# TinyMPC/TinyMPC

Hardware: AMD Instinct MI355X
Metric: QP solves/sec (+ ADMM iters/sec), 64k-batch quadrotor hover (higher is better)
Workload: dtype f64; 1 GPU; quadrotor_hovering (nx=12, nu=4, N=10), 65536 identical instances per GPU, closed-loop MPC steps from a cold start (BASELINE configs[1]); batch_per_gpu=65536, total_batch=65536, parallelism=batch-sharded x1, mpc_steps_per_launch=8, stats_exchange=none (one rank), launcher=plain process

## Files before the change

### tinympc_amd/csrc/admm_kernel.hip.h

```cpp
#pragma once
#include <hip/hip_runtime.h>
#include <stdint.h>

namespace tinympc_amd {

enum : int {
    TAB_MB = 0,
    TAB_MF1 = 256,
    TAB_MF2 = 512,
    TAB_PT = 768,
    TAB_VEC = 1024,
    TAB_BOUNDS = 1024 + 16 * 16,
};
enum : int {
    VEC_CB = 0,
    VEC_CF = 1,
    VEC_QR = 2,
    VEC_SMASK = 3,
    VEC_NIM = 4,
    VEC_SOCFLAG = 5,
    VEC_CONE_BASE = 6,
    VEC_CONE_MU = 7,
    VEC_LINFLAG = 9,
    VEC_TLINFLAG = 10,
// ... 385 lines not shown
#define HAH7 HAH6 "v_fmac_f64_dpp %[acc], %[sa], %[a6] row_newbcast:8+6 row_mask:0xf bank_mask:0xc\n\t"
#define HAH8 HAH7 "v_fmac_f64_dpp %[acc], %[sa], %[a7] row_newbcast:8+7 row_mask:0xf bank_mask:0xc\n\t"
#define HBL1 "v_fmac_f64_dpp %[acc], %[sb], %[b0] row_newbcast:%[c0]+0 row_mask:0xf bank_mask:0x3\n\t"
#define HBL2 HBL1 "v_fmac_f64_dpp %[acc], %[sb], %[b1] row_newbcast:%[c0]+1 row_mask:0xf bank_mask:0x3\n\t"
#define HBL3 HBL2 "v_fmac_f64_dpp %[acc], %[sb], %[b2] row_newbcast:%[c0]+2 row_mask:0xf bank_mask:0x3\n\t"
#define HBL4 HBL3 "v_fmac_f64_dpp %[acc], %[sb], %[b3] row_newbcast:%[c0]+3 row_mask:0xf bank_mask:0x3\n\t"
#define HBL5 HBL4 "v_fmac_f64_dpp %[acc], %[sb], %[b4] row_newbcast:%[c0]+4 row_mask:0xf bank_mask:0x3\n\t"
#define HBL6 HBL5 "v_fmac_f64_dpp %[acc], %[sb], %[b5] row_newbcast:%[c0]+5 row_mask:0xf bank_mask:0x3\n\t"
#define HBL7 HBL6 "v_fmac_f64_dpp %[acc], %[sb], %[b6] row_newbcast:%[c0]+6 row_mask:0xf bank_mask:0x3\n\t"
#define HBL8 HBL7 "v_fmac_f64_dpp %[acc], %[sb], %[b7] row_newbcast:%[c0]+7 row_mask:0xf bank_mask:0x3\n\t"
#define HBH1 "v_fmac_f64_dpp %[acc], %[sb], %[b0] row_newbcast:8+%[c0]+0 row_mask:0xf bank_mask:0xc\n\t"
#define HBH2 HBH1 "v_fmac_f64_dpp %[acc], %[sb], %[b1] row_newbcast:8+%[c0]+1 row_mask:0xf bank_mask:0xc\n\t"
#define HBH3 HBH2 "v_fmac_f64_dpp %[acc], %[sb], %[b2] row_newbcast:8+%[c0]+2 row_mask:0xf bank_mask:0xc\n\t"
#define HBH4 HBH3 "v_fmac_f64_dpp %[acc], %[sb], %[b3] row_newbcast:8+%[c0]+3 row_mask:0xf bank_mask:0xc\n\t"
#define HBH5 HBH4 "v_fmac_f64_dpp %[acc], %[sb], %[b4] row_newbcast:8+%[c0]+4 row_mask:0xf bank_mask:0xc\n\t"
#define HBH6 HBH5 "v_fmac_f64_dpp %[acc], %[sb], %[b5] row_newbcast:8+%[c0]+5 row_mask:0xf bank_mask:0xc\n\t"
#define HBH7 HBH6 "v_fmac_f64_dpp %[acc], %[sb], %[b6] row_newbcast:8+%[c0]+6 row_mask:0xf bank_mask:0xc\n\t"
#define HBH8 HBH7 "v_fmac_f64_dpp %[acc], %[sb], %[b7] row_newbcast:8+%[c0]+7 row_mask:0xf bank_mask:0xc\n\t"
#define HFAL1 "v_fmac_f64_dpp %[t], %[xi], %[a0] row_newbcast:0 row_mask:0xf bank_mask:0x3\n\t"
#define HFAL2 HFAL1 "v_fmac_f64_dpp %[t], %[xi], %[a1] row_newbcast:1 row_mask:0xf bank_mask:0x3\n\t"
#define HFAL3 HFAL2 "v_fmac_f64_dpp %[t], %[xi], %[a2] row_newbcast:2 row_mask:0xf bank_mask:0x3\n\t"
#define HFAL4 HFAL3 "v_fmac_f64_dpp %[t], %[xi], %[a3] row_newbcast:3 row_mask:0xf bank_mask:0x3\n\t"
#define HFAL5 HFAL4 "v_fmac_f64_dpp %[t], %[xi], %[a4] row_newbcast:4 row_mask:0xf bank_mask:0x3\n\t"
#define HFAL6 HFAL5 "v_fmac_f64_dpp %[t], %[xi], %[a5] row_newbcast:5 row_mask:0xf bank_mask:0x3\n\t"
#define HFAL7 HFAL6 "v_fmac_f64_dpp %[t], %[xi], %[a6] row_newbcast:6 row_mask:0xf bank_mask:0x3\n\t"
#define HFAL8 HFAL7 "v_fmac_f64_dpp %[t], %[xi], %[a7] row_newbcast:7 row_mask:0xf bank_mask:0x3\n\t"
#define HFAH1 "v_fmac_f64_dpp %[t], %[xi], %[a0] row_newbcast:8+0 row_mask:0xf bank_mask:0xc\n\t"
#define HFAH2 HFAH1 "v_fmac_f64_dpp %[t], %[xi], %[a1] row_newbcast:8+1 row_mask:0xf bank_mask:0xc\n\t"
#define HFAH3 HFAH2 "v_fmac_f64_dpp %[t], %[xi], %[a2] row_newbcast:8+2 row_mask:0xf bank_mask:0xc\n\t"
#define HFAH4 HFAH3 "v_fmac_f64_dpp %[t], %[xi], %[a3] row_newbcast:8+3 row_mask:0xf bank_mask:0xc\n\t"
#define HFAH5 HFAH4 "v_fmac_f64_dpp %[t], %[xi], %[a4] row_newbcast:8+4 row_mask:0xf bank_mask:0xc\n\t"
#define HFAH6 HFAH5 "v_fmac_f64_dpp %[t], %[xi], %[a5] row_newbcast:8+5 row_mask:0xf bank_mask:0xc\n\t"
#define HFAH7 HFAH6 "v_fmac_f64_dpp %[t], %[xi], %[a6] row_newbcast:8+6 row_mask:0xf bank_mask:0xc\n\t"
#define HFAH8 HFAH7 "v_fmac_f64_dpp %[t], %[xi], %[a7] row_newbcast:8+7 row_mask:0xf bank_mask:0xc\n\t"
#define HFBL1 "v_fmac_f64_dpp %[xn], %[t], %[b0] row_newbcast:%[c0]+0 row_mask:0xf bank_mask:0x3\n\t"
#define HFBL2 HFBL1 "v_fmac_f64_dpp %[xn], %[t], %[b1] row_newbcast:%[c0]+1 row_mask:0xf bank_mask:0x3\n\t"
#define HFBL3 HFBL2 "v_fmac_f64_dpp %[xn], %[t], %[b2] row_newbcast:%[c0]+2 row_mask:0xf bank_mask:0x3\n\t"
#define HFBL4 HFBL3 "v_fmac_f64_dpp %[xn], %[t], %[b3] row_newbcast:%[c0]+3 row_mask:0xf bank_mask:0x3\n\t"
#define HFBL5 HFBL4 "v_fmac_f64_dpp %[xn], %[t], %[b4] row_newbcast:%[c0]+4 row_mask:0xf bank_mask:0x3\n\t"
#define HFBL6 HFBL5 "v_fmac_f64_dpp %[xn], %[t], %[b5] row_newbcast:%[c0]+5 row_mask:0xf bank_mask:0x3\n\t"
#define HFBL7 HFBL6 "v_fmac_f64_dpp %[xn], %[t], %[b6] row_newbcast:%[c0]+6 row_mask:0xf bank_mask:0x3\n\t"
#define HFBL8 HFBL7 "v_fmac_f64_dpp %[xn], %[t], %[b7] row_newbcast:%[c0]+7 row_mask:0xf bank_mask:0x3\n\t"
#define HFBH1 "v_fmac_f64_dpp %[xn], %[t], %[b0] row_newbcast:8+%[c0]+0 row_mask:0xf bank_mask:0xc\n\t"
#define HFBH2 HFBH1 "v_fmac_f64_dpp %[xn], %[t], %[b1] row_newbcast:8+%[c0]+1 row_mask:0xf bank_mask:0xc\n\t"
#define HFBH3 HFBH2 "v_fmac_f64_dpp %[xn], %[t], %[b2] row_newbcast:8+%[c0]+2 row_mask:0xf bank_mask:0xc\n\t"
#define HFBH4 HFBH3 "v_fmac_f64_dpp %[xn], %[t], %[b3] row_newbcast:8+%[c0]+3 row_mask:0xf bank_mask:0xc\n\t"
#define HFBH5 HFBH4 "v_fmac_f64_dpp %[xn], %[t], %[b4] row_newbcast:8+%[c0]+4 row_mask:0xf bank_mask:0xc\n\t"
#define HFBH6 HFBH5 "v_fmac_f64_dpp %[xn], %[t], %[b5] row_newbcast:8+%[c0]+5 row_mask:0xf bank_mask:0xc\n\t"
#define HFBH7 HFBH6 "v_fmac_f64_dpp %[xn], %[t], %[b6] row_newbcast:8+%[c0]+6 row_mask:0xf bank_mask:0xc\n\t"
#define HFBH8 HFBH7 "v_fmac_f64_dpp %[xn], %[t], %[b7] row_newbcast:8+%[c0]+7 row_mask:0xf bank_mask:0xc\n\t"
#define FUSED_HBWD_CASE(NA_, NB_) FUSED_HBWD_CASE_(NA_, NB_)
#define FUSED_HBWD_CASE_(NA_, NB_)                                                                                      \
    if constexpr (NA == NA_ && NB == NB_) {                                                                             \
        asm("v_fma_f64 %[qlo], -%[rho], %[tmp], %[qx]\n\t"                                                              \
            "v_fma_f64 %[acc], %[qlo], %[smask], %[cb]\n\t"                                                             \
            "v_fma_f64 %[dnp], %[sa], %[nim], %[cf]\n\t" HAL##NA_ HBL##NB_                                              \
            "v_add_f64 %[tmpn], %[vnn], -%[gn]\n\t" HAH##NA_ HBH##NB_                                                   \
            : [qlo] "=&v"(qlo), [acc] "=&v"(acc), [dnp] "=&v"(dnp), [tmpn] "=&v"(tmpn)                                  \
            : [tmp] "v"(tmp), [vnn] "v"(vnn), [gn] "v"(gn), [qx] "v"(qx), [rho] "v"(rho), [smask] "v"(smask), [cb] "v"(cb), \
              [nim] "v"(nim), [cf] "v"(cf), [sa] "v"(sa), [sb] "v"(sb), [c0] "i"(NA_), FMA##NA_, FMB##NB_);             \
    }
#define FUSED_HFWD_CASE(NA_, NB_) FUSED_HFWD_CASE_(NA_, NB_)
#define FUSED_HFWD_CASE_(NA_, NB_)                                                                                      \
    if constexpr (NA == NA_ && NB == NB_) {                                                                             \
        asm("v_add_f64 %[tt], %[xi], %[g]\n\t"                                                                          \
            "v_max_f64 %[vm], %[lo], %[tt]\n\t" HFAL##NA_                                                               \
            "v_min_f64 %[vn], %[hi], %[vm]\n\t" HFAH##NA_                                                               \
            "v_mov_b64 %[xn], %[t]\n\t"                                                                                 \
            "v_add_f64 %[gnew], %[tt], -%[vn]\n\t" HFBL##NB_                                                            \
            "s_nop 0\n\t" HFBH##NB_                                                                                     \
            : [tt] "=&v"(tt), [vm] "=&v"(vm), [vn] "=&v"(vn), [xn] "=&v"(xn), [t] "+&v"(t), [gnew] "=&v"(gnew)           \
            : [xi] "v"(xi), [g] "v"(g), [lo] "v"(lo), [hi] "v"(hi), [c0] "i"(NA_), FMA##NA_, FMB##NB_);                  \
    }
#if defined(TINYMPC_FUSED_NX) && defined(TINYMPC_FUSED_NU)
#define FUSED_SHAPES(CASE) CASE(TINYMPC_FUSED_NX, TINYMPC_FUSED_NU)
constexpr bool fused_shape(int na, int nb) { return na == TINYMPC_FUSED_NX && nb == TINYMPC_FUSED_NU; }
#if TINYMPC_FUSED_NX + TINYMPC_FUSED_NU <= 8
#define FUSED_HALF_SHAPES(CASE) CASE(TINYMPC_FUSED_NX, TINYMPC_FUSED_NU)
#else
#define FUSED_HALF_SHAPES(CASE)
#endif
#else
#define FUSED_SHAPES(CASE)
#define FUSED_HALF_SHAPES(CASE)
constexpr bool fused_shape(int, int) { return false; }
#endif
template <int NA, int NB>
__device__ __forceinline__ void fused_backward_step(double& qlo, double& acc, double vn, double g, double qx, double rho, double smask, double cb,
                                                    double sa, double sb, const double* ma, const double* mb_) {
    double tmp;
    FUSED_SHAPES(FUSED_BWD_CASE)
    (void)tmp;
}
template <int NA, int NB>
__device__ __forceinline__ void fused_backward_step_soc(double& qlo, double& acc, double vn, double g, double qx, double w, double rho,
                                                        double smask, double cb, double sa, double sb, const double* ma, const double* mb_) {
    double tmp;
    FUSED_SHAPES(FUSED_BWD_SOC_CASE)
    (void)tmp;
}
template <int NA, int NB>
__device__ __forceinline__ void fused_backward_step_half(double& qlo, double& acc, double& dnp, double& tmpn, double tmp, double vnn, double gn, double qx,
                                                         double rho, double smask, double cb, double nim, double cf, double sa, double sb,
                                                         const double* ma, const double* mb_) {
    FUSED_HALF_SHAPES(FUSED_HBWD_CASE)
}
template <int NA, int NB>
__device__ __forceinline__ void fused_forward_step_half(double& tt, double& vn, double& t, double& xn, double& gnew, double xi, double g,
                                                        double lo, double hi, const double* ma, const double* mb_) {
    double vm;
    FUSED_HALF_SHAPES(FUSED_HFWD_CASE)
    (void)vm;
}
template <int NA, int NB, bool INPLACE = false>
__device__ __forceinline__ void fused_forward_step(double& tt, double& vn, double& t, double& xn, double xi, double g, double lo, double hi,
                                                   const double* ma, const double* mb_) {
    double vm;
    FUSED_SHAPES(FUSED_FWD_CASE)
    (void)vm;
}

__device__ __forceinline__ double vmax64(double a, double b) {
    double r;
    asm("v_max_f64 %0, %1, %2" : "=v"(r) : "v"(a), "v"(b));
    return r;
}
__device__ __forceinline__ double vmin64(double a, double b) {
    double r;
    asm("v_min_f64 %0, %1, %2" : "=v"(r) : "v"(a), "v"(b));
    return r;
}
__device__ __forceinline__ double pinned_sub64(double a, double b) {
    double r = a - b;
    asm volatile("" : "+v"(r));
    return r;
}
__device__ __forceinline__ double vclamp64(double lo, double hi, double t) {
    double r;
    asm("v_max_f64 %0, %1, %2\n\tv_min_f64 %0, %3, %0" : "=&v"(r) : "v"(lo), "v"(t), "v"(hi));
    return r;
}

__device__ __forceinline__ double vmax_abs64(double a, double b) {
    double r;
    asm("v_max_f64 %0, %1, |%2|" : "=v"(r) : "v"(a), "v"(b));
    return r;
}
template <bool OPAQUE>
__device__ __forceinline__ double resid_max(double a, double b) {
    if constexpr (OPAQUE) return vmax_abs64(a, b);
    else return fmax(a, fabs(b));
}

#ifndef TINYMPC_PRIM_STORE
#define TINYMPC_PRIM_STORE 1
#endif
#ifndef TINYMPC_REF_LOAD
#define TINYMPC_REF_LOAD 1
#endif
#ifndef TINYMPC_FULL_LINE_STORES
#define TINYMPC_FULL_LINE_STORES 2
#endif
__device__ __forceinline__ double load_ref(const double* p) {
#if TINYMPC_REF_LOAD == 1
    return __builtin_nontemporal_load(p);
#else
    return *p;
#endif
}
__device__ __forceinline__ void store_primal(double* p, double v) {
#if TINYMPC_PRIM_STORE == 1
    __builtin_nontemporal_store(v, p);
#elif TINYMPC_PRIM_STORE == 2
    asm volatile("global_store_dwordx2 %0, %1, off sc1" : : "v"(p), "v"(v) : "memory");
#elif TINYMPC_PRIM_STORE == 3
    asm volatile("global_store_dwordx2 %0, %1, off sc0 sc1" : : "v"(p), "v"(v) : "memory");
#elif TINYMPC_PRIM_STORE == 4
    asm volatile("global_store_dwordx2 %0, %1, off sc0 sc1 nt" : : "v"(p), "v"(v) : "memory");
#else
    *p = v;
#endif
}

__device__ __forceinline__ double grp_max16(double v) {
#pragma unroll
    for (int off = 8; off >= 1; off >>= 1) v = fmax(v, __shfl_xor(v, off, 16));
    return v;
}
template <int W>
__device__ __forceinline__ double grp_maxw(double v) {
#pragma unroll
    for (int off = W / 2; off >= 1; off >>= 1) v = fmax(v, __shfl_xor(v, off, W));
    return v;
}

__device__ __forceinline__ double soc_component(double s0, double s1, double s2, double mine, int c, float mu) {
#pragma clang fp contract(off)
    const double u0 = s2 * (double)mu;
    const double q0 = s0 * s0, q1 = s1 * s1;
    const double q = q0 + q1;
    const bool sure_inside = (u0 > 1e-30) && (q <= (u0 * u0) * (1.0 - 0x1p-20)) && (q < 1e70);
    if (__builtin_amdgcn_ballot_w64(!sure_inside) == 0ull) return mine;
    const float a = (float)sqrt(q);
    const double ad = (double)a;
    const bool below = ad <= -u0, inside = ad <= u0;
    const bool outside = !below && !inside && (ad >= fabs(u0));
    double r = (below || !inside) ? 0.0 : mine;
    if (__builtin_amdgcn_ballot_w64(outside) != 0ull) {
        const double scale = 0.5 * (1.0 + u0 / ad);
        const double last = (double)(a / mu);
        const double o = scale * ((c == 2) ? last : mine);
        r = outside ? o : r;
    }
    return r;
}

__device__ __forceinline__ bool soc_all_inside(double s0, double s1, double s2, float mu) {
#pragma clang fp contract(off)
    const double u0 = s2 * (double)mu;
    const double q0 = s0 * s0, q1 = s1 * s1;
    const double q = q0 + q1;
    const bool sure_inside = (u0 > 1e-30) & (u0 < 1e300) & (q <= (u0 * u0) * (1.0 - 0x1p-20)) & (q < 1e70);
    return __builtin_amdgcn_ballot_w64(!sure_inside) == 0ull;
}
__device__ __forceinline__ void soc_project3(double s0, double s1, double s2, float mu, float rmu, bool rmu_exact, double& r0, double& r1, double& r2) {
#pragma clang fp contract(off)
    const double u0 = s2 * (double)mu;
    const double q0 = s0 * s0, q1 = s1 * s1;
    const double q = q0 + q1;
    const float a = (float)sqrt(q);
    const double ad = (double)a;
    const bool below = ad <= -u0, inside = ad <= u0;
    const bool outside = !below && !inside && (ad >= fabs(u0));
    const bool zero = below || !inside;
    r0 = zero ? 0.0 : s0; r1 = zero ? 0.0 : s1; r2 = zero ? 0.0 : s2;
    if (__builtin_amdgcn_ballot_w64(outside) != 0ull) {
        const double scale = 0.5 * (1.0 + u0 / ad);
        const double last = (double)(rmu_exact ? a * rmu : a / mu);
        r0 = outside ? scale * s0 : r0;
        r1 = outside ? scale * s1 : r1;
        r2 = outside ? scale * last : r2;
    }
}
__device__ __forceinline__ int soc_items_of(unsigned heads, int nx, int n) {
    int c = 0;
    for (unsigned m = heads; m; m &= m - 1) c += (__builtin_ctz(m) < nx) ? n : n - 1;
    return c;
}
constexpr int soc_item_passes(int nx, int nu, int n) { return ((nx / 3) * n + (nu / 3) * (n - 1) + 15) / 16; }

constexpr int ADAPT_LOG = 32;
__device__ __forceinline__ double taylor_step(double a, double d, double b) {
#pragma clang fp contract(off)
    const double t = d * b;
    return a + t;
}

constexpr int solve_kernel_waves_per_simd(int nz, int n, bool soc, bool lin = false, bool adapt = false) {
    if (lin) return 1;
    if (adapt) return n <= 10 ? 2 : 1;
    return (n <= 10 || 2 * ((soc ? 8 : 6) * n + 2 * nz + 8) + 40 <= 256) ? 2 : 1;
}

#ifndef TINYMPC_LIN_WAVES
#define TINYMPC_LIN_WAVES 0
#endif
constexpr long solve_kernel_lin_lds(int nx, int nu, int n, bool soc, int lin, int kmax, bool ub) {
    const int nz = nx + nu, csl = (nz + 1) | 1, cs = (nz + 1) | 1;
    return 8L * (nx * 16 + (ub ? 2 : 2 * n * 16) + ((lin & 1) ? 3 * kmax * 16 + 2 * 4 * n * csl : 0) +
                 ((lin & 2) ? 3 * n * kmax * 16 + 2 * 4 * n * csl : 0) + (soc ? (4 * n + 1) * 3 * cs : 0));
}
constexpr bool solve_kernel_lin_planes(int nx, int nu, int n, bool soc, int lin, int kmax, bool ub) {
    return lin != 0 && solve_kernel_lin_lds(nx, nu, n, soc, lin, kmax, ub) <= 64 * 1024 - 512;
}
constexpr int solve_kernel_lin_waves(int nx, int nu, int n, bool soc, int lin, int kmax, bool ub) {
    if (!solve_kernel_lin_planes(nx, nu, n, soc, lin, kmax, ub)) return 1;
    if (TINYMPC_LIN_WAVES > 0) return TINYMPC_LIN_WAVES;
    return (solve_kernel_waves_per_simd(nx + nu, n, soc) == 2 && 8 * solve_kernel_lin_lds(nx, nu, n, soc, lin, kmax, ub) <= 158 * 1024) ? 2 : 1;
}
template <int NF, int KMAX_, int LW_, int LPI_>
__device__ __forceinline__ void project_halfspace_columns(const int t, const int inst, const int n, const int csl, const int R0, const int S0,
                                                          double* pv, double* pg, const double* tab, const int tab_stride, const int nk) {
#pragma clang fp contract(off)
    for (int c = S0 + t; c < n; c += LPI_) {
        const int at = (inst * n + c) * csl + R0;
        const double* tk = tab + c * tab_stride;
        double z[NF], t0[NF];
#pragma unroll
        for (int r = 0; r < NF; ++r) { z[r] = pv[at + r]; t0[r] = z[r]; }
        for (int k = 0; k < nk; ++k) {
            double cv = 0.0;
#pragma unroll
            for (int r = 0; r < NF; ++r) { const double pr = tk[k * LW_ + R0 + r] * z[r]; cv = cv + pr; }
            const double bk = tk[KMAX_ * LW_ + k * LW_ + R0];
            if (cv > bk) {
                const double dist = (cv - bk) / tk[2 * KMAX_ * LW_ + k * LW_ + R0];
#pragma unroll
                for (int r = 0; r < NF; ++r) { const double pr = dist * tk[k * LW_ + R0 + r]; z[r] = z[r] - pr; }
            }
        }
#pragma unroll
        for (int r = 0; r < NF; ++r) { pv[at + r] = z[r]; pg[at + r] = t0[r] - z[r]; }
    }
}

template <int NX, int NU, int N, bool SOC, bool DBG, int MODE, int LIN = 0, bool HET = false, int KMAX = LIN_KMAX, bool ADAPT = false, bool UB = false, bool HALF = false,
// ... 274 lines not shown
            const int cw = grp * N * SLOT_D + (j < NZ ? j : NZ);
            const double x0v_in = is_state ? (PF ? pf_x0 : P.x0[(size_t)b * NX + j]) : 0.0;
            const int cl = grp * N * CSL + (j < NZ ? j : NZ);
            double VL[LSR ? N : 1], GL[LSR ? N : 1], VT[LTR ? N : 1], GT[LTR ? N : 1];
            double Qd[DBG ? N : 1], Pd[DBG ? N : 1], Dd[DBG ? N : 1];
            double ref_last = 0.0, qx_last_plain = 0.0;
#pragma unroll
            for (int s = 0; s < N; ++s) {
                const bool valid = is_state || (is_input && s >= 1);
                const size_t off = lbase + s * NZ;
                const bool warm = valid && !P.cold;
                if constexpr (PF) {
                    VN[s] = warm ? pfVN[s] : 0.0;
                    G[s] = warm ? pfG[s] : 0.0;
                    VP[s] = warm ? pfVP[s] : 0.0;
                    QX[s] = pfQXs[s];
                    X[s] = 0.0;
                    if (s == N - 1) ref_last = pf_rl;
                    continue;
                }
                const double r = valid ? (P.ref_shared ? P.ref[off - (size_t)b * (N * NZ)] : load_ref(P.ref + off)) : 0.0;
                VN[s] = warm ? P.slack[off] : 0.0;
                G[s] = warm ? P.dual[off] : 0.0;
                VP[s] = warm ? P.slack_prev[off] : 0.0;
                QX[s] = -(r * qr);
                X[s] = 0.0;
                if (s == N - 1) ref_last = r;
                if constexpr (SOC) {
                    double vc0 = (warm && soc_lane) ? (resumed ? P.cslack : P.prim)[off] : 0.0;
                    const double gc0 = (warm && soc_lane) ? P.cdual[off] : 0.0;
                    if (s == 0 && is_state && soc_lane && !resumed) vc0 = x0v_in;
                    sC[cw + s * SLOT_D] = vc0 - gc0;
                    sC[cw + s * SLOT_D + PL_GC] = gc0;
                    sC[cw + s * SLOT_D + PL_VC] = vc0;
                }
                if constexpr (LS) {
                    const double vl0 = (warm && lin_lane) ? (resumed ? P.lslack : P.prim)[off] : 0.0;
                    const double gl0 = (warm && lin_lane) ? P.ldual[off] : 0.0;
                    if constexpr (LSP) { sLV[cl + s * CSL] = vl0; sLG[cl + s * CSL] = gl0; } else { VL[s] = vl0; GL[s] = gl0; }
                }
                if constexpr (LT) {
                    const double vt0 = (warm && tlin_lane) ? (resumed ? P.tlslack : P.prim)[off] : 0.0;
                    const double gt0 = (warm && tlin_lane) ? P.tldual[off] : 0.0;
                    if constexpr (LTP) { sTV[cl + s * CSL] = vt0; sTG[cl + s * CSL] = gt0; } else { VT[s] = vt0; GT[s] = gt0; }
                }
                if constexpr (DBG) { Qd[s] = 0.0; Pd[s] = 0.0; Dd[s] = 0.0; }
            }
            double x0v = x0v_in;
            auto terminal_term = [&]() {
                double pt[NX];
#pragma unroll
                for (int k = 0; k < NX; ++k)
                    pt[k] = ADAPT ? sP[grp * NX * NX + k + NX * (is_state ? j : 0)] : (HET ? het[TAB_PT + k * 16 + j] : sPt[k * 16 + j]);
                double xp = 0.0;
                if constexpr (HALF) ring1_half<0, NX>(xp, ref_last, pt);
                else xp = ring_sum<MODE, 0, NX>(0.0, ref_last, pt);
                qx_last_plain = QX[N - 1];
                QX[N - 1] = is_state ? -xp : QX[N - 1];
            };
            int ndl = 0;
            auto flush_c = [&](int n) {
                __builtin_amdgcn_fence(__ATOMIC_RELEASE, "wavefront");
                __builtin_amdgcn_wave_barrier();
                if (P.aC2 && is_state) {
                    double* c2 = P.aC2 + (size_t)b * (NX * NX) + NX * j;
                    double v[NX], d[NX];
#pragma unroll
                    for (int k = 0; k < NX; ++k) { v[k] = c2[k]; d[k] = P.atab[ATAB_DC2 + k * 16 + j]; }
                    for (int i = 0; i < n; ++i) {
                        const double dl = sDl[grp * ADAPT_LOG + i];
#pragma unroll
                        for (int k = 0; k < NX; ++k) v[k] = taylor_step(v[k], dl, d[k]);
                    }
#pragma unroll
                    for (int k = 0; k < NX; ++k) c2[k] = v[k];
                }
                if (P.aC1 && j < NU) {
                    double* c1 = P.aC1 + (size_t)b * (NU * NU) + NU * j;
                    double v[NU], d[NU];
#pragma unroll
                    for (int k = 0; k < NU; ++k) { v[k] = c1[k]; d[k] = P.atab[ATAB_DC1 + k * 16 + j]; }
                    for (int i = 0; i < n; ++i) {
                        const double dl = sDl[grp * ADAPT_LOG + i];
#pragma unroll
                        for (int k = 0; k < NU; ++k) v[k] = taylor_step(v[k], dl, d[k]);
                    }
#pragma unroll
                    for (int k = 0; k < NU; ++k) c1[k] = v[k];
                }
            };
            if (!has_traj && !(PF && P.ref_shared)) terminal_term();
            const int traj_k0 = has_traj ? (P.traj_step0 + (P.traj_offsets ? P.traj_offsets[b] : 0)) : 0;

            int iter = 0, solved = 0, checked = 0;
            unsigned acc_iter = 0, acc_solved = 0;
            bool vp_touched = false;
            double rp = 0.0, rd = 0.0;
            const int nsteps = PF ? 1 : (P.steps > 1 ? P.steps : 1);
            const int iter_first = resumed ? P.iter_base : 0;
            for (int step = 0; step < nsteps; ++step) {
                X[0] = x0v;
                if (has_traj) {
                    if (is_state) {
#pragma unroll
                        for (int s = 0; s < N; ++s) {
                            int kk = traj_k0 + step + s;
                            kk = kk < P.traj_points ? kk : P.traj_points - 1;
                            const double r = P.traj[(size_t)kk * NX + j];
                            QX[s] = -(r * qr);
                            if (s == N - 1) ref_last = r;
                        }
                    }
                    terminal_term();
                }
                if (P.reset_duals) {
#pragma unroll
                    for (int s = 0; s < N; ++s) G[s] = 0.0;
                }
                if constexpr (SOC) {
                    if (step > 0) {
#pragma unroll
                        for (int s = 0; s < N; ++s) {
                            const double vc0 = soc_lane ? X[s] : 0.0;
                            sC[cw + s * SLOT_D] = vc0 - sC[cw + s * SLOT_D + PL_GC];
                            sC[cw + s * SLOT_D + PL_VC] = vc0;
                        }
                    }
                }
                if constexpr (LS) {
                    if (step > 0) {
#pragma unroll
                        for (int s = 0; s < N; ++s) { if constexpr (LSP) sLV[cl + s * CSL] = lin_lane ? X[s] : 0.0; else VL[s] = lin_lane ? X[s] : 0.0; }
                    } else if (is_state && lin_lane && !resumed) { if constexpr (LSP) sLV[cl] = x0v; else VL[0] = x0v; }
                }
                if constexpr (LT) {
                    if (step > 0) {
#pragma unroll
                        for (int s = 0; s < N; ++s) { if constexpr (LTP) sTV[cl + s * CSL] = tlin_lane ? X[s] : 0.0; else VT[s] = tlin_lane ? X[s] : 0.0; }
                    } else if (is_state && tlin_lane && !resumed) { if constexpr (LTP) sTV[cl] = x0v; else VT[0] = x0v; }
                }
                if constexpr (LPL) __builtin_amdgcn_fence(__ATOMIC_RELEASE, "wavefront");
                const int iter0 = iter_first;
                iter = iter0; solved = 0;
                if (resumed && P.check_termination > 0) checked = 1;
                int countdown = P.check_termination;
                double wr[SOC ? SPR : 1];
                bool gcz[SOC_PASSES];
#pragma unroll
                for (int p = 0; p < SOC_PASSES; ++p) gcz[p] = false;
                if constexpr (SOC) {
#pragma unroll
                    for (int d = 1; d <= SPR && d <= N; ++d) wr[(N - d) % SPR] = sC[cw + (N - d) * SLOT_D];
                }
                for (int it = iter0; it < P.max_iter; ++it) {
                    double lvr[LSP ? SPR : 1], lgr[LSP ? SPR : 1], tvr[LTP ? SPR : 1], tgr[LTP ? SPR : 1];
                    if constexpr (LPL) {
#pragma unroll
                        for (int d = 1; d <= SPR && d <= N; ++d) {
                            if constexpr (LSP) { lvr[(N - d) % SPR] = sLV[cl + (N - d) * CSL]; lgr[(N - d) % SPR] = sLG[cl + (N - d) * CSL]; }
                            if constexpr (LTP) { tvr[(N - d) % SPR] = sTV[cl + (N - d) * CSL]; tgr[(N - d) % SPR] = sTG[cl + (N - d) * CSL]; }
                        }
                    }
                    auto lin_w = [&](const int s_) { if constexpr (LSP) return lvr[s_ % SPR] - lgr[s_ % SPR]; else return VL[LSR ? s_ : 0] - GL[LSR ? s_ : 0]; };
                    auto tlin_w = [&](const int s_) { if constexpr (LTP) return tvr[s_ % SPR] - tgr[s_ % SPR]; else return VT[LTR ? s_ : 0] - GT[LTR ? s_ : 0]; };
                    double qhi;
                    {
                        double t = fma(-rho, VN[N - 1] - G[N - 1], QX[N - 1]);
                        if constexpr (SOC) t = fma(-rho, wr[(N - 1) % SPR], t);
                        if constexpr (LS) t = fma(-rho, lin_w(N - 1), t);
                        if constexpr (LT) t = fma(-rho, tlin_w(N - 1), t);
                        qhi = t;
                        if constexpr (DBG) {
                            double ql = fma(-rho, VN[N - 1] - G[N - 1], qx_last_plain);
                            if constexpr (SOC) ql = fma(-rho, wr[(N - 1) % SPR], ql);
                            if constexpr (LS) ql = fma(-rho, lin_w(N - 1), ql);
                            if constexpr (LT) ql = fma(-rho, tlin_w(N - 1), ql);
                            Qd[N - 1] = is_state ? ql : t;
                            Pd[N - 1] = t;
                        }
                    }
                    double pcur = qhi;
                    if constexpr (HALF) {
                        double tmpv = VN[N - 2] - G[N - 2];
#pragma unroll
                        for (int i = N - 2; i >= 0; --i) {
                            double qlo, res, dnp, tmpn;
                            constexpr int dummy = 0;
                            const int in = i > 0 ? i - 1 : dummy;
                            fused_backward_step_half<NX, NU>(qlo, res, dnp, tmpn, tmpv, VN[in], G[in], QX[i], rho, smask, cb, nim, cf, pcur, qhi, mb, mb + NX);
                            if (i + 1 <= N - 2) Dn[i + 1] = dnp;
                            tmpv = tmpn;
                            pcur = res;
                            qhi = qlo;
                        }
                        Dn[0] = fma(pcur, nim, cf);
                    }
#pragma unroll
                    for (int i = N - 2; i >= 0 && !HALF; --i) {
                        if constexpr (SOC) {
                            if (i >= SPD) wr[(i - SPD) % SPR] = sC[cw + (i - SPD) * SLOT_D];
                        }
                        if constexpr (LSP) { if (i >= SPD) { lvr[(i - SPD) % SPR] = sLV[cl + (i - SPD) * CSL]; lgr[(i - SPD) % SPR] = sLG[cl + (i - SPD) * CSL]; } }
                        if constexpr (LTP) { if (i >= SPD) { tvr[(i - SPD) % SPR] = sTV[cl + (i - SPD) * CSL]; tgr[(i - SPD) % SPR] = sTG[cl + (i - SPD) * CSL]; } }
                        if constexpr (SOC || LPL) __builtin_amdgcn_sched_barrier(0);
                        if constexpr (FUSED) {
                            double qlo, res;
                            if constexpr (SOC) fused_backward_step_soc<NX, NU>(qlo, res, VN[i], G[i], QX[i], wr[i % SPR], rho, smask, cb, pcur, qhi, mb, mb + NX);
                            else fused_backward_step<NX, NU>(qlo, res, VN[i], G[i], QX[i], rho, smask, cb, pcur, qhi, mb, mb + NX);
                            pcur = res;
                            Dn[i] = fma(res, nim, cf);
                            if constexpr (DBG) { Qd[i] = qlo; Pd[i] = res; Dd[i + 1] = res; }
                            qhi = qlo;
                            continue;
                        }
                        double qlo = fma(-rho, VN[i] - G[i], QX[i]);
                        if constexpr (SOC) qlo = fma(-rho, wr[i % SPR], qlo);
                        if constexpr (LS) qlo = fma(-rho, lin_w(i), qlo);
                        if constexpr (LT) qlo = fma(-rho, tlin_w(i), qlo);
                        const double res = ring_sum2<MODE, NX, NU>(fma(qlo, smask, cb), pcur, mb, qhi, mb + NX);
                        pcur = res;
                        Dn[i] = fma(res, nim, cf);
                        if constexpr (DBG) { Qd[i] = qlo; Pd[i] = res; Dd[i + 1] = res; }
                        qhi = qlo;
                    }
                    constexpr bool LAZY_RES = N <= 12;
                    constexpr bool TIGHT = FUSED && !HALF && LAZY_RES && !SOC && NX % 4 == 0;
                    double pmax = 0.0, dmax = 0.0;
                    auto slot_update = [&](const int s, const double lo, const double hi, const double gcv, const double glv, const double gtv) {
                        const double xi = X[s];
                        const double t = xi + G[s];
                        const double vn = TIGHT ? vclamp64(lo, hi, t) : vmin64(hi, vmax64(lo, t));
                        if constexpr (!LAZY_RES) {
                            pmax = resid_max<true>(pmax, xi - vn);
                            dmax = resid_max<true>(dmax, VP[s] - vn);
                        }
                        G[s] = t - vn;
                        VN[s] = vn;
                        if constexpr (SOC) {
                            sC[cw + s * SLOT_D] = fma(xi, socmask, gcv);
                        }
                        if constexpr (LSP) sLV[cl + s * CSL] = (lin_lane && (is_state || s >= 1)) ? (xi + glv) : 0.0;
                        if constexpr (LTP) sTV[cl + s * CSL] = (tlin_lane && (is_state || s >= 1)) ? (xi + gtv) : 0.0;
                        if constexpr (LSR || LTR) {
                            auto halfspaces = [&](double z, const double* tabk, const int nk) {
                                for (int k = 0; k < nk; ++k) {
                                    const double a = tabk[k * 16 + j];
                                    const double bk = tabk[KMAX * 16 + k * 16 + j];
                                    const double nn = tabk[2 * KMAX * 16 + k * 16 + j];
                                    const double prod = a * z;
                                    double cs = 0.0, ci = 0.0;
                                    ring1<0, NX>(cs, prod, ones);
                                    ring1<NX, NU>(ci, prod, ones);
                                    const double cv = is_state ? cs : ci;
                                    if (cv > bk) z = z - ((cv - bk) / nn) * a;
                                }
                                return z;
                            };
                            if constexpr (LSR) {
                                const bool on = lin_lane && (is_state || s >= 1);
                                double vl = on ? (xi + GL[s]) : 0.0;
                                vl = halfspaces(vl, sLin, P.n_lin);
                                GL[s] = on ? ((GL[s] + xi) - vl) : 0.0;
                                VL[s] = on ? vl : 0.0;
                            }
                            if constexpr (LTR) {
                                const bool on = tlin_lane && (is_state || s >= 1);
                                double vt = on ? (xi + GT[s]) : 0.0;
                                vt = halfspaces(vt, sTLin + s * 3 * KMAX * 16, P.n_tlin);
                                GT[s] = on ? ((GT[s] + xi) - vt) : 0.0;
                                VT[s] = on ? vt : 0.0;
                            }
                        }
                    };
                    double lo_c = UB ? lo_u0 : sLo[j], hi_c = UB ? hi_u0 : sHi[j];
                    double gr[SOC ? SPR : 1];
                    if constexpr (SOC) {
#pragma unroll
                        for (int d = 0; d < SPD && d < N; ++d) gr[d % SPR] = sC[cw + d * SLOT_D + PL_GC];
                    } else gr[0] = 0.0;
                    double glr[LSP ? SPR : 1], gtr[LTP ? SPR : 1];
                    glr[0] = 0.0; gtr[0] = 0.0;
                    if constexpr (LPL) {
#pragma unroll
                        for (int d = 0; d < SPD && d < N; ++d) {
                            if constexpr (LSP) glr[d % SPR] = sLG[cl + d * CSL];
                            if constexpr (LTP) gtr[d % SPR] = sTG[cl + d * CSL];
                        }
                    }
                    double tt_d = 0.0, vn_d = 0.0;
#pragma unroll
                    for (int i = 0; i < N - 1; ++i) {
                        const double lo_n = UB ? lo_u : sLo[(i + 1) * 16 + j], hi_n = UB ? hi_u : sHi[(i + 1) * 16 + j];
                        if constexpr (SOC) { if (i + SPD < N) gr[(i + SPD) % SPR] = sC[cw + (i + SPD) * SLOT_D + PL_GC]; }
                        if constexpr (LSP) { if (i + SPD < N) glr[(i + SPD) % SPR] = sLG[cl + (i + SPD) * CSL]; }
                        if constexpr (LTP) { if (i + SPD < N) gtr[(i + SPD) % SPR] = sTG[cl + (i + SPD) * CSL]; }
                        __builtin_amdgcn_sched_barrier(0);
                        if constexpr (FUSED) {
                            double tt, vn, xn, t = Dn[i];
                            const double xi = X[i];
                            if constexpr (HALF) {
                                double gnew;
                                fused_forward_step_half<NX, NU>(tt, vn, t, xn, gnew, xi, G[i], lo_c, hi_c, mf1, mf2);
                                X[i + 1] = xn;
                                if constexpr (!LAZY_RES) {
                                    pmax = resid_max<true>(pmax, xi - vn);
                                    dmax = resid_max<true>(dmax, VP[i] - vn);
                                }
                                G[i] = gnew;
                                VN[i] = vn;
                                lo_c = lo_n; hi_c = hi_n;
                                continue;
                            }
                            fused_forward_step<NX, NU, TIGHT>(tt, vn, t, xn, xi, G[i], lo_c, hi_c, mf1, mf2);
                            X[i + 1] = xn;
                            if constexpr (!LAZY_RES) {
                                pmax = resid_max<true>(pmax, xi - vn);
                                dmax = resid_max<true>(dmax, VP[i] - vn);
                            }
                            if constexpr (TIGHT) {
                                __builtin_amdgcn_sched_barrier(0);
                                if (i > 0) G[i - 1] = pinned_sub64(tt_d, vn_d);
                                tt_d = tt; vn_d = vn;
                            } else G[i] = tt - vn;
                            VN[i] = vn;
                            if constexpr (SOC) sC[cw + i * SLOT_D] = fma(xi, socmask, gr[i % SPR]);
                            lo_c = lo_n; hi_c = hi_n;
                            continue;
                        }
                        const double t = ring_sum<MODE, 0, NX>(Dn[i], X[i], mf1);
                        X[i + 1] = ring_short<MODE, NX, NU>(t, t, mf2);
                        slot_update(i, lo_c, hi_c, gr[SOC ? i % SPR : 0], glr[LSP ? i % SPR : 0], gtr[LTP ? i % SPR : 0]);
                        lo_c = lo_n; hi_c = hi_n;
                    }
                    if constexpr (TIGHT && N >= 2) G[N - 2] = tt_d - vn_d;
                    (void)tt_d; (void)vn_d;
                    slot_update(N - 1, lo_c, hi_c, gr[SOC ? (N - 1) % SPR : 0], glr[LSP ? (N - 1) % SPR : 0], gtr[LTP ? (N - 1) % SPR : 0]);
                    if constexpr (LPL) {
                        __builtin_amdgcn_fence(__ATOMIC_RELEASE, "wavefront");
                        __builtin_amdgcn_wave_barrier();
                        if constexpr (LSP) {
                            if (lin_x_on) project_halfspace_columns<NX, KMAX, 16, 16>(j, grp, N, CSL, 0, 0, sLV, sLG, sLin, 0, P.n_lin);
                            if (lin_u_on) project_halfspace_columns<NU, KMAX, 16, 16>(j, grp, N, CSL, NX, 1, sLV, sLG, sLin, 0, P.n_lin);
                        }
                        if constexpr (LTP) {
                            if (tlin_x_on) project_halfspace_columns<NX, KMAX, 16, 16>(j, grp, N, CSL, 0, 0, sTV, sTG, sTLin, 3 * KMAX * 16, P.n_tlin);
                            if (tlin_u_on) project_halfspace_columns<NU, KMAX, 16, 16>(j, grp, N, CSL, NX, 1, sTV, sTG, sTLin, 3 * KMAX * 16, P.n_tlin);
                        }
                        __builtin_amdgcn_fence(__ATOMIC_RELEASE, "wavefront");
                        __builtin_amdgcn_wave_barrier();
                    }
                    bool conv = false;
                    auto termination = [&]() {
                        if (countdown > 0 && --countdown == 0) {
                            countdown = P.check_termination;
                            checked = 1;
                            constexpr int PS0 = N >= 2 ? 1 : 0, PS1 = N - 1;
                            auto lost = [&](const int s) {
                                return (int)(fabs(X[s] - VN[s]) >= P.tol_pri) | (int)(fabs(VP[s] - VN[s]) * rho >= P.tol_dua);
                            };
                            const bool maybe = ((int)!(rho > 0.0) | (int)!(lost(PS0) | lost(PS1))) != 0;
                            unsigned long long fold = __ballot(maybe);
                            fold &= fold >> 1; fold &= fold >> 2; fold &= fold >> 4;
                            if constexpr (!HALF) fold &= fold >> 8;
                            const bool any_row = (fold & (HALF ? 0x0101010101010101ull : 0x0001000100010001ull)) != 0ull;
                            const bool last_test = (P.max_iter - 1 - it) < P.check_termination;
                            if (last_test || any_row) {
                                if constexpr (LAZY_RES) {
#pragma unroll
                                    for (int s = 0; s < N; ++s) {
                                        pmax = resid_max<false>(pmax, X[s] - VN[s]);
                                        dmax = resid_max<false>(dmax, VP[s] - VN[s]);
                                    }
                                }
                                rp = pmax;
                                rd = dmax * rho;
                                const bool ok = (rp < P.tol_pri) && (rd < P.tol_dua);
                                const unsigned long long bal = __ballot(ok);
                                conv = ((bal >> (grp * RL)) & RMASK) == RMASK;
                            }
                        }
                    };
                    if constexpr (SOC) {
                        __builtin_amdgcn_fence(__ATOMIC_RELEASE, "wavefront");
                        __builtin_amdgcn_wave_barrier();
                        double n0 = sC[item_at[0]], n1 = sC[item_at[0] + 1], n2 = sC[item_at[0] + 2];
#pragma unroll
                        for (int d = 1; d <= SPR && d <= N; ++d) wr[(N - d) % SPR] = sC[cw + (N - d) * SLOT_D];
                        termination();
                        bool any_exact = false;
#pragma unroll
                        for (int p = 0; p < SOC_PASSES; ++p) {
                            if (p > 0 && p >= soc_passes) break;
                            const int at = item_at[p];
                            if (p > 0) { n0 = sC[at]; n1 = sC[at + 1]; n2 = sC[at + 2]; }
                            const double s0 = n0, s1 = n1, s2 = n2;
                            if (soc_all_inside(s0, s1, s2, item_mu[p])) {
                                sC[at + PL_VC] = s0; sC[at + PL_VC + 1] = s1; sC[at + PL_VC + 2] = s2;
                                if (!gcz[p]) {
                                    sC[at + PL_GC] = 0.0; sC[at + PL_GC + 1] = 0.0; sC[at + PL_GC + 2] = 0.0;
                                    gcz[p] = true;
                                }
                            } else {
                                double r0, r1, r2;
                                soc_project3(s0, s1, s2, item_mu[p], item_rmu[p], mu_pow2, r0, r1, r2);
                                const double g0 = s0 - r0, g1 = s1 - r1, g2 = s2 - r2;
                                sC[at + PL_VC] = r0; sC[at + PL_VC + 1] = r1; sC[at + PL_VC + 2] = r2;
                                sC[at + PL_GC] = g0; sC[at + PL_GC + 1] = g1; sC[at + PL_GC + 2] = g2;
                                sC[at] = r0 - g0; sC[at + 1] = r1 - g1; sC[at + 2] = r2 - g2;
                                gcz[p] = false;
                                any_exact = true;
                            }
                        }
                        if (it == iter0 && !proj_lane) {
#pragma unroll
                            for (int s = 0; s < N; ++s) sC[cw + s * SLOT_D + PL_GC] = 0.0;
                        }
                        __builtin_amdgcn_fence(__ATOMIC_RELEASE, "wavefront");
                        __builtin_amdgcn_wave_barrier();
                        if (any_exact) {
#pragma unroll
                            for (int d = 1; d <= SPR && d <= N; ++d) wr[(N - d) % SPR] = sC[cw + (N - d) * SLOT_D];
                        }
                    }
                    iter += 1;
                    if constexpr (ADAPT) {
                        if (it > 0 && it % 5 == 0) {
                            double at[NX];
#pragma unroll
                            for (int k = 0; k < NX; ++k) at[k] = sTab[j * AKC + k];
                            double pri_res = 0.0, ax_max = 0.0, z_max = 0.0, dual_res = 0.0, px_max = 0.0, aty_max = 0.0, q_max = 0.0;
                            double pxq_max = 0.0;
#pragma unroll
                            for (int i = 0; i < N - 1; ++i) {
                                const double axs = ring_sum<MODE, 0, NX>(0.0, X[i], mf1);
                                const double dyn = ring_short<MODE, NX, NU>(axs, is_input ? X[i + 1] : 0.0, mf2) - X[i + 1];
                                const double a = is_state ? dyn : X[i + 1];
                                const double zz = VN[i + 1];
                                const bool on = is_state || is_input;
                                pri_res = fmax(pri_res, on ? fabs(a - zz) : 0.0);
                                ax_max = fmax(ax_max, on ? fabs(a) : 0.0);
                                z_max = fmax(z_max, on ? fabs(zz) : 0.0);
                                const double init = is_state ? (i >= 1 ? -G[i] : 0.0) : G[i + 1];
                                const double aty = ring_sum<MODE, 0, NX>(init, G[i + 1], at);
                                const double xs = is_state ? X[i] : X[i + 1];
                                const double px = qr * xs;
                                dual_res = fmax(dual_res, on ? fabs((px + px) + aty) : 0.0);
                                pxq_max = fmax(pxq_max, on ? fabs(px) : 0.0);
                                aty_max = fmax(aty_max, on ? fabs(aty) : 0.0);
                            }
                            {
                                double prow[NX];
#pragma unroll
                                for (int k = 0; k < NX; ++k) prow[k] = sP[grp * NX * NX + (is_state ? j : 0) + NX * k];
                                const double pxl = ring_sum<MODE, 0, NX>(0.0, X[N - 1], prow);
                                const double ql = qr * X[N - 1];
                                const double atyl = -G[N - 1];
                                dual_res = fmax(dual_res, is_state ? fabs((pxl + ql) + atyl) : 0.0);
                                px_max = fmax(pxq_max, is_state ? fabs(pxl) : 0.0);
                                aty_max = fmax(aty_max, is_state ? fabs(atyl) : 0.0);
                                q_max = fmax(pxq_max, is_state ? fabs(ql) : 0.0);
                            }
                            pri_res = grp_max16(pri_res); ax_max = grp_max16(ax_max); z_max = grp_max16(z_max);
                            dual_res = grp_max16(dual_res); px_max = grp_max16(px_max); aty_max = grp_max16(aty_max); q_max = grp_max16(q_max);
                            const double pri_norm = fmax(ax_max, z_max);
                            const double dual_norm = fmax(fmax(px_max, aty_max), q_max);
                            const double eps = 1e-10;
                            const double normalized_pri = pri_res / (pri_norm + eps);
                            const double normalized_dual = dual_res / (dual_norm + eps);
                            const double ratio = normalized_pri / (normalized_dual + eps);
                            double new_rho = rho * sqrt(ratio);
                            if (P.aclip) new_rho = fmin(fmax(new_rho, P.arho_min), P.arho_max);
                            const double delta = new_rho - rho;
                            if (is_state) {
#pragma unroll
                                for (int k = 0; k < NU; ++k) mb[NX + k] = -taylor_step(-mb[NX + k], delta, sTab[(16 + j) * AKC + k]);
#pragma unroll
                                for (int k = 0; k < NX; ++k) {
                                    const int e = grp * NX * NX + k + NX * j;
                                    sP[e] = taylor_step(sP[e], delta, sTab[(32 + j) * AKC + k]);
                                }
                            } else if (is_input) {
#pragma unroll
                                for (int k = 0; k < NX; ++k) mf1[k] = -taylor_step(-mf1[k], delta, sTab[(16 + j) * AKC + k]);
                            }
                            if (P.aC1 || P.aC2) {
                                if (j == 0) sDl[grp * ADAPT_LOG + ndl] = delta;
                                if (++ndl == ADAPT_LOG) { flush_c(ndl); ndl = 0; }
                            }
                            rho = new_rho;
                            __builtin_amdgcn_fence(__ATOMIC_RELEASE, "wavefront");
                            __builtin_amdgcn_wave_barrier();
                            QX[N - 1] = qx_last_plain;
                            terminal_term();
                        }
                    }
                    if constexpr (!SOC) termination();
                    if (conv) { solved = 1; break; }
#pragma unroll
                    for (int s = 0; s < N; ++s) VP[s] = VN[s];
                    vp_touched = true;
                }
                acc_iter += (unsigned)(iter - iter0);
                acc_solved += (unsigned)solved;
                if (P.iter_log && j == 0) P.iter_log[(size_t)step * P.batch + b] = solved ? iter : -iter;
                if (P.u0_log && is_input) P.u0_log[((size_t)step * P.batch + b) * NU + (j - NX)] = X[1];
                if (nsteps > 1) {
                    x0v = is_state ? X[1] : 0.0;
                }
            }

            constexpr bool FLS = TINYMPC_FULL_LINE_STORES != 0 && (PF || TINYMPC_FULL_LINE_STORES == 2) && !SOC && LIN == 0 && !DBG;
            if (FLS && (P.store_mask & 32) == 0) {
                if constexpr (FLS) {
                    const size_t seg = (size_t)b * (N * NZ) + j;
                    const bool in_row = j < NZ;
#pragma unroll
                    for (int s = 0; s < N; ++s) {
                        const size_t off = seg + s * NZ;
                        const double xs = is_input ? (s + 1 < N ? X[s + 1 < N ? s + 1 : s] : 0.0) : X[s];
                        const double vs = is_input ? (s + 1 < N ? VN[s + 1 < N ? s + 1 : s] : 0.0) : VN[s];
                        const double gs = is_input ? (s + 1 < N ? G[s + 1 < N ? s + 1 : s] : 0.0) : G[s];
                        const double ps = is_input ? (s + 1 < N ? VP[s + 1 < N ? s + 1 : s] : 0.0) : VP[s];
                        if (in_row) {
                            if (P.store_mask & 1) {
                                if (acc_iter > 0) { if constexpr (PF) P.prim[off] = xs; else store_primal(P.prim + off, xs); }
                                else if (s == 0 && is_state) P.prim[off] = xs;
                            }
                            if (P.store_mask & 2) P.slack[off] = vs;
                            if (P.store_mask & 4) P.dual[off] = gs;
                            if ((P.store_mask & 8) && vp_touched) P.slack_prev[off] = ps;
                        }
                    }
                }
            } else
#pragma unroll
            for (int s = 0; s < N; ++s) {
                const bool valid = is_state || (is_input && s >= 1);
                const size_t off = lbase + s * NZ;
                if (valid) {
                    if (((P.store_mask & 1) || ((P.store_mask & 32) && s <= 1)) && (acc_iter > 0 || (s == 0 && is_state))) {
                        if constexpr (SOC || LIN != 0) P.prim[off] = X[s];
                        else store_primal(P.prim + off, X[s]);
                    }
                    if (P.store_mask & 2) P.slack[off] = VN[s];
                    if (P.store_mask & 4) P.dual[off] = G[s];
                    if ((P.store_mask & 8) && vp_touched) P.slack_prev[off] = VP[s];
                    if constexpr (SOC) {
                        if (soc_lane && (P.store_mask & 16)) {
                            P.cslack[off] = sC[cw + s * SLOT_D + ((proj_lane || iter <= iter_first) ? PL_VC : 0)];
                            P.cdual[off] = sC[cw + s * SLOT_D + PL_GC];
                        }
                    }
                    if constexpr (LSP) { if (lin_lane && (P.store_mask & 16)) { P.lslack[off] = sLV[cl + s * CSL]; P.ldual[off] = sLG[cl + s * CSL]; } }
                    if constexpr (LTP) { if (tlin_lane && (P.store_mask & 16)) { P.tlslack[off] = sTV[cl + s * CSL]; P.tldual[off] = sTG[cl + s * CSL]; } }
                    if constexpr (LSR) { if (lin_lane && (P.store_mask & 16)) { P.lslack[off] = VL[s]; P.ldual[off] = GL[s]; } }
                    if constexpr (LTR) { if (tlin_lane && (P.store_mask & 16)) { P.tlslack[off] = VT[s]; P.tldual[off] = GT[s]; } }
                    if constexpr (DBG) {
                        if (P.dbg_qr && acc_iter > 0) {
                            P.dbg_qr[off] = Qd[s];
                            P.dbg_pd[off] = is_state ? Pd[s] : Dd[s];
                        }
                    }
                }
            }
            if constexpr (ADAPT) {
                if (ndl > 0) flush_c(ndl);
                if (j == 0) P.arho[b] = rho;
                if (is_state) {
#pragma unroll
                    for (int k = 0; k < NU; ++k) P.aK[(size_t)b * (NU * NX) + k + NU * j] = -mb[NX + k];
#pragma unroll
                    for (int k = 0; k < NX; ++k) P.aP[(size_t)b * (NX * NX) + k + NX * j] = sP[grp * NX * NX + k + NX * j];
                }
            }
            if (P.x0_next && acc_iter > 0 && is_state) P.x0_next[(size_t)b * NX + j] = X[1];
            const double ps = grp_maxw<RL>(is_state ? rp : 0.0), pi = grp_maxw<RL>(is_input ? rp : 0.0);
            const double ds = grp_maxw<RL>(is_state ? rd : 0.0), di = grp_maxw<RL>(is_input ? rd : 0.0);
            if (P.next_index) {
                const bool open = j == 0 && !solved;
                const unsigned long long m = __ballot(open);
                if (m) {
                    const int first = __ffsll((long long)m) - 1;
                    int at = 0;
                    if (lane == first) at = atomicAdd(P.next_count, __popcll(m));
                    at = __shfl(at, first);
                    if (open) P.next_index[at + __popcll(m & ((1ull << lane) - 1ull))] = b;
                }
            }
            if (j == 0) {
                P.status[b] = make_int4(iter, solved, solved ? 1 : 11, checked);
                double4 rr = make_double4(ps, pi, ds, di);
                *reinterpret_cast<double4*>(P.resid + (size_t)b * 4) = rr;
                if (P.accum) {
                    if constexpr (PF) {
                        __hip_atomic_fetch_add(&P.accum[b].x, acc_iter, __ATOMIC_RELAXED, __HIP_MEMORY_SCOPE_AGENT);
                        __hip_atomic_fetch_add(&P.accum[b].y, acc_solved, __ATOMIC_RELAXED, __HIP_MEMORY_SCOPE_AGENT);
                    } else {
                        uint2 ac = P.accum[b];
                        ac.x += acc_iter;
                        ac.y += acc_solved;
                        P.accum[b] = ac;
                    }
                }
            }
        }
    }
}

}
```

Measured before the change: 2.885 billion QP solves/s.

## Add lean ADMM loop with sparse termination checks and skipped slack copies

For fused, non-SOC, non-adaptive full-wave configurations, the ADMM iteration loop is restructured into an inner do-while that runs until the next termination check. Residual tests use cheaper wave ballots with a bit-trick zero-group detector. The previous-slack copy (VP=VN) is done only on the iteration right before a check instead of every iteration. The goal is to cut per-iteration bookkeeping: the countdown, the iteration counter, the slack copy and the lambda-based termination. In exchange, iteration counting and convergence flags are reconstructed after the loop, which risks subtle mismatches in the iteration count and in the solved/checked semantics.

```diff
diff --git a/tinympc_amd/csrc/admm_kernel.hip.h b/tinympc_amd/csrc/admm_kernel.hip.h
--- a/tinympc_amd/csrc/admm_kernel.hip.h
+++ b/tinympc_amd/csrc/admm_kernel.hip.h
@@ -561,6 +561,10 @@
     else return fmax(a, fabs(b));
 }
 
+__device__ __forceinline__ bool zero_group16(const unsigned long long w) {
+    return ((w - 0x0001000100010001ull) & ~w & 0x8000800080008000ull) != 0ull;
+}
+
 #ifndef TINYMPC_PRIM_STORE
 #define TINYMPC_PRIM_STORE 1
 #endif
@@ -1141,7 +1145,15 @@
 #pragma unroll
                     for (int d = 1; d <= SPR && d <= N; ++d) wr[(N - d) % SPR] = sC[cw + (N - d) * SLOT_D];
                 }
+                constexpr bool LEAN = FUSED && !HALF && N <= 12 && !SOC && NX % 4 == 0 && !ADAPT && !HET;
+                [[maybe_unused]] int next_test = P.check_termination > 0 ? iter0 + P.check_termination - 1 : 0x7fffffff;
+                [[maybe_unused]] int full_from = rho > 0.0 ? P.max_iter - P.check_termination : (int)0x80000000;
+                if constexpr (LEAN) asm("" : "+s"(full_from));
+                [[maybe_unused]] unsigned long long ok_lanes = 0ull;
                 for (int it = iter0; it < P.max_iter; ++it) {
+                    bool conv = false;
+                    [[maybe_unused]] int limit = P.max_iter;
+                    do {
                     double lvr[LSP ? SPR : 1], lgr[LSP ? SPR : 1], tvr[LTP ? SPR : 1], tgr[LTP ? SPR : 1];
                     if constexpr (LPL) {
 #pragma unroll
@@ -1338,7 +1350,7 @@
                         __builtin_amdgcn_fence(__ATOMIC_RELEASE, "wavefront");
                         __builtin_amdgcn_wave_barrier();
                     }
-                    bool conv = false;
+                    conv = false;
                     auto termination = [&]() {
                         if (countdown > 0 && --countdown == 0) {
                             countdown = P.check_termination;
@@ -1411,7 +1423,7 @@
                             for (int d = 1; d <= SPR && d <= N; ++d) wr[(N - d) % SPR] = sC[cw + (N - d) * SLOT_D];
                         }
                     }
-                    iter += 1;
+                    if constexpr (!LEAN) iter += 1;
                     if constexpr (ADAPT) {
                         if (it > 0 && it % 5 == 0) {
                             double at[NX];
@@ -1483,11 +1495,46 @@
                             terminal_term();
                         }
                     }
-                    if constexpr (!SOC) termination();
-                    if (conv) { solved = 1; break; }
+                    if constexpr (LEAN) {
+                        if (it == next_test) {
+                            next_test += P.check_termination;
+                            constexpr int PS0 = N >= 2 ? 1 : 0, PS1 = N - 1;
+                            const double pri = fmax(fabs(X[PS0] - VN[PS0]), fabs(X[PS1] - VN[PS1]));
+                            const double dua = fmax(fabs(VP[PS0] - VN[PS0]), fabs(VP[PS1] - VN[PS1])) * rho;
+                            const unsigned long long out = ~__builtin_amdgcn_read_exec();
+                            const unsigned long long not_maybe = __builtin_amdgcn_ballot_w64(pri >= P.tol_pri) |
+                                                                 __builtin_amdgcn_ballot_w64(dua >= P.tol_dua) | out;
+                            if (zero_group16(it >= full_from ? 0ull : not_maybe)) {
+#pragma unroll
+                                for (int s = 0; s < N; ++s) {
+                                    pmax = resid_max<false>(pmax, X[s] - VN[s]);
+                                    dmax = resid_max<false>(dmax, VP[s] - VN[s]);
+                                }
+                                rp = pmax;
+                                rd = dmax * rho;
+                                ok_lanes = __builtin_amdgcn_ballot_w64((rp < P.tol_pri) && (rd < P.tol_dua));
+                                if (zero_group16(~ok_lanes | out)) limit = it + 1;
+                            }
+                        }
+                        if (it + 1 == next_test && it + 1 < limit) {
+#pragma unroll
+                            for (int s = 0; s < N; ++s) VP[s] = VN[s];
+                        }
+                    } else if constexpr (!SOC) termination();
+                    } while (LEAN && ++it < limit);
+                    if constexpr (LEAN) {
+                        --it;
+                        conv = ((ok_lanes >> (grp * RL)) & RMASK) == RMASK;
+                    }
+                    if (conv) { if constexpr (LEAN) iter = it + 1; solved = 1; break; }
 #pragma unroll
                     for (int s = 0; s < N; ++s) VP[s] = VN[s];
-                    vp_touched = true;
+                    if constexpr (!LEAN) vp_touched = true;
+                    if constexpr (LEAN) { if (it + 1 >= P.max_iter) { iter = it + 1; break; } }
+                }
+                if constexpr (LEAN) {
+                    if (P.check_termination > 0 && iter - iter0 >= P.check_termination) checked = 1;
+                    if (iter - iter0 > solved) vp_touched = true;
                 }
                 acc_iter += (unsigned)(iter - iter0);
                 acc_solved += (unsigned)solved;
```

Result: slower. 2.760 billion QP solves/s (median of 2 runs) (-4.3%).
